# okieraised/rs-face-detection-tflite

Hardware: AMD Instinct MI355X
Metric: faces/sec at batch=256 (256x256 back-camera) per GPU (higher is better)
Workload: dtype f32

## Files before the change

### rs-face-detection-tflite_amd/csrc/chain_kernels.hip

```cpp
#include <hip/hip_runtime.h>

#include <algorithm>
#include <cstdint>
#include <type_traits>

#include "kernels.hpp"
#include "launch.hpp"

namespace mi {

typedef float f32x16c __attribute__((ext_vector_type(16)));
typedef float f32x2c __attribute__((ext_vector_type(2)));
typedef float f32x4c __attribute__((ext_vector_type(4)));

namespace {

__device__ __forceinline__ float4 cld4(const float* p) { return *reinterpret_cast<const float4*>(p); }

struct ChainGeom {
    int Cp, Ch, C4, PS, RS, MT;
    int off_wdw, off_bdw, off_bias, off_alpha;
    int split;
    int pre_P, pre_RP, pre_GP, pre_PS, pre_RS;
    int off_t8;
    int lds_bytes;
    unsigned long long* stamps;
};
#ifdef MI_CHAIN_STAMPS
unsigned long long* g_chain_stamps = nullptr;
#define MI_CHAIN_STAMP(k) if (g.stamps && threadIdx.x == 0) { __builtin_amdgcn_sched_barrier(0); g.stamps[(long)blockIdx.x * 24 + (k)] = __builtin_amdgcn_s_memtime(); __builtin_amdgcn_sched_barrier(0); }
#else
#define MI_CHAIN_STAMP(k)
#endif

constexpr int chain_pre_passes(int C, int H, int W, int Cin, int post_Co, int MT, bool split, long tile) {
    const int pre_RS = (2 * W + 1) * (Cin + 4);
    for (int P = 1; P <= 4; P++) {
        const int RP = (H + P - 1) / P, GP = (RP * W + 31) / 32;
        const long stage = (long)(2 * RP + 1) * pre_RS;
        const long rest = 9 * C + C + 8 * 32 + 64 + (post_Co ? (long)(H >> 1) * (W >> 1) * (post_Co + 4) : 0);
        if ((P - 1) * RP < H && P * GP * (split ? MT : 1) <= 8 && ((stage > tile ? stage : tile) + rest) * 4 <= 160 * 1024 - 256) return P;
    }
    return 0;
}

struct GeomRun {
    [[maybe_unused]] static constexpr bool fixed = false;
    static constexpr bool all_res = false;
    const ChainArgs& a;
    const ChainGeom& g;
    __device__ GeomRun(const ChainArgs& a_, const ChainGeom& g_) : a(a_), g(g_) {}
    __device__ int C() const { return a.C; }
    __device__ int H() const { return a.H; }
    __device__ int W() const { return a.W; }
    __device__ int pre_on() const { return a.pre.on; }
    __device__ int pre_Cin() const { return a.pre.Cin; }
    __device__ int post_on() const { return a.post.on; }
    __device__ int post_Co() const { return a.post.Co; }
#define MI_GEOM_FIELD(f) __device__ int f() const { return g.f; }
    MI_GEOM_FIELD(Cp) MI_GEOM_FIELD(Ch) MI_GEOM_FIELD(C4) MI_GEOM_FIELD(PS) MI_GEOM_FIELD(RS)
    MI_GEOM_FIELD(off_wdw) MI_GEOM_FIELD(off_bdw) MI_GEOM_FIELD(off_bias) MI_GEOM_FIELD(off_alpha)
    MI_GEOM_FIELD(pre_P) MI_GEOM_FIELD(pre_RP) MI_GEOM_FIELD(pre_GP) MI_GEOM_FIELD(pre_PS) MI_GEOM_FIELD(pre_RS)
#undef MI_GEOM_FIELD
};
template <int C_, int H_, int W_, int CIN, int CO>
struct GeomFixed {
    static constexpr bool fixed = true;
    static constexpr bool all_res = true;
    struct K {
        static constexpr int C = C_, H = H_, W = W_, Cp = C, Ch = C / 2, C4 = C / 4, PS = C + 4, RS = (W + 2) * PS, MT = (C + 31) / 32;
        static constexpr bool split = MT > 1 && ((H * W + 31) / 32) * MT <= 8;
        static constexpr int pre_on = CIN != 0, pre_Cin = CIN, post_on = CO != 0, post_Co = CO;
        static constexpr int tile = (H + 2) * RS;
        static constexpr int pre_PS = CIN + 4, pre_RS = (2 * W + 1) * pre_PS;
        static constexpr int pre_P = CIN ? chain_pre_passes(C, H, W, CIN, CO, MT, split, tile) : 0;
        static constexpr int pre_RP = CIN ? (H + pre_P - 1) / pre_P : 0, pre_GP = (pre_RP * W + 31) / 32;
        static constexpr int stage = CIN ? (2 * pre_RP + 1) * pre_RS : 0;
        static constexpr int off_wdw = stage > tile ? stage : tile, off_bdw = off_wdw + 9 * Cp, off_bias = (off_bdw + Cp + 3) & ~3;
        static constexpr int off_alpha = off_bias + MT * 32;
    };
    static_assert(!CIN || K::pre_P > 0, "no staging plan for `pre`");
    __device__ GeomFixed(const ChainArgs&, const ChainGeom&) {}
#define MI_GEOM_FIELD(f) static constexpr __device__ int f() { return K::f; }
    MI_GEOM_FIELD(C) MI_GEOM_FIELD(H) MI_GEOM_FIELD(W) MI_GEOM_FIELD(pre_on) MI_GEOM_FIELD(pre_Cin) MI_GEOM_FIELD(post_on) MI_GEOM_FIELD(post_Co)
    MI_GEOM_FIELD(Cp) MI_GEOM_FIELD(Ch) MI_GEOM_FIELD(C4) MI_GEOM_FIELD(PS) MI_GEOM_FIELD(RS)
    MI_GEOM_FIELD(off_wdw) MI_GEOM_FIELD(off_bdw) MI_GEOM_FIELD(off_bias) MI_GEOM_FIELD(off_alpha)
    MI_GEOM_FIELD(pre_P) MI_GEOM_FIELD(pre_RP) MI_GEOM_FIELD(pre_GP) MI_GEOM_FIELD(pre_PS) MI_GEOM_FIELD(pre_RS)
#undef MI_GEOM_FIELD
    static bool matches(const ChainArgs& a, const ChainGeom& g) {
        bool ok = a.C == K::C && a.H == K::H && a.W == K::W && g.Cp == K::Cp && g.Ch == K::Ch && g.C4 == K::C4 && g.PS == K::PS && g.RS == K::RS &&
                  g.MT == K::MT && (g.split != 0) == K::split && g.off_wdw == K::off_wdw && g.off_bdw == K::off_bdw && g.off_bias == K::off_bias &&
                  g.off_alpha == K::off_alpha && (a.pre.on != 0) == (CIN != 0) && (a.post.on != 0) == (CO != 0);
        if (ok && CIN) ok = a.pre.Cin == CIN && g.pre_P == K::pre_P && g.pre_RP == K::pre_RP && g.pre_GP == K::pre_GP && g.pre_PS == K::pre_PS && g.pre_RS == K::pre_RS;
        if (ok && CO) ok = a.post.Co == CO;
        for (int k = 0; ok && k < a.nblocks; k++) ok = a.blocks[k].has_res != 0;
        return ok;
    }
};
constexpr int kActRun = -1;

struct DwTaps { f32x4c w[9], d[9], b; };
template <int WS_, int RSB_, int PSB_, bool BIAS_FIRST_>
struct DwForm { static constexpr int WS = WS_, RSB = RSB_, PSB = PSB_; static constexpr bool bias_first = BIAS_FIRST_; };
template <int OFF>
__device__ __forceinline__ void lds_request(unsigned addr, f32x4c& v) { asm volatile("ds_read_b128 %0, %1 offset:%2" : "=v"(v) : "v"(addr), "n"(OFF)); }
template <class F, int... K>
__device__ __forceinline__ void dw_request(unsigned wa, unsigned ta, DwTaps& t, std::integer_sequence<int, K...>) {
    static_assert(9 * F::WS + 16 * 16 < 65536 && 2 * F::RSB + 2 * F::PSB + 16 * 16 < 65536, "ds_read offsets are 16 bits");
    ((lds_request<K * F::WS>(wa, t.w[K]), lds_request<(K / 3) * F::RSB + (K % 3) * F::PSB>(ta, t.d[K])), ...);
    lds_request<9 * F::WS>(wa, t.b);
}
template <class F>
__device__ __forceinline__ void dw_request(unsigned wa, unsigned ta, DwTaps& t) { dw_request<F>(wa, ta, t, std::make_integer_sequence<int, 9>{}); }
__device__ __forceinline__ void dw_landed(DwTaps& t) {
    asm volatile("s_waitcnt lgkmcnt(0)" ::: "memory");
#pragma unroll
    for (int k = 0; k < 9; k++) asm volatile("" : "+v"(t.w[k]), "+v"(t.d[k]));
    asm volatile("" : "+v"(t.b));
}
template <bool BIAS_FIRST>
__device__ __forceinline__ void dw_fma(const DwTaps& t, float4& bf) {
    f32x2c lo = {0.f, 0.f}, up = {0.f, 0.f};
    if constexpr (BIAS_FIRST) { lo = f32x2c{t.b.x, t.b.y}; up = f32x2c{t.b.z, t.b.w}; }
#pragma unroll
    for (int k = 0; k < 9; k++) {
        lo = __builtin_elementwise_fma(f32x2c{t.d[k].x, t.d[k].y}, f32x2c{t.w[k].x, t.w[k].y}, lo);
        up = __builtin_elementwise_fma(f32x2c{t.d[k].z, t.d[k].w}, f32x2c{t.w[k].z, t.w[k].w}, up);
    }
    if constexpr (!BIAS_FIRST) { lo += f32x2c{t.b.x, t.b.y}; up += f32x2c{t.b.z, t.b.w}; }
    asm volatile("" : "+v"(lo), "+v"(up));
    bf = make_float4(lo.x, lo.y, up.x, up.y);
}

template <int MT, bool SPLIT, class GP = GeomRun, int ACT = kActRun, int SCHED = 0>
__global__ __launch_bounds__(512, 2) void chain_kernel(ChainArgs a, ChainGeom g) {
    extern __shared__ __attribute__((aligned(16))) float lds[];
    const GP geo(a, g);
    float* tile = lds;
    const int tid = threadIdx.x, lane = tid & 63, wave = tid >> 6;
    const int pl = lane & 31, h = lane >> 5;
    const int b = blockIdx.x;
    const float* in = a.in + (long)b * a.in_fs;
    const int rowf4 = geo.W() * geo.C4();
    const int nch = geo.Ch() >> 2;

    struct ConstRegs { float w[3], bdw, bias, alpha; };
    auto fetch_consts = [&](const ChainBlock& cb, int Cs, int Cos, ConstRegs& r) {
#pragma unroll
        for (int k = 0; k < 3; k++) {
            const int i = tid + 512 * k, c = i % geo.Cp();
            r.w[k] = (i < 9 * geo.Cp() && c < Cs) ? cb.w_dw[(i / geo.Cp()) * Cs + c] : 0.f;
        }
        r.bdw = (tid < Cs && cb.b_dw) ? cb.b_dw[tid] : 0.f;
        r.bias = (tid < Cos && cb.bias) ? cb.bias[tid] : 0.f;
        if constexpr (ACT == kActRun) r.alpha = (tid < Cos && cb.act == ACT_PRELU) ? cb.alpha[tid] : (cb.act == ACT_NONE ? 1.f : 0.f);
    };
    auto commit_consts = [&](const ConstRegs& r) {
#pragma unroll
        for (int k = 0; k < 3; k++)
            if (tid + 512 * k < 9 * geo.Cp()) lds[geo.off_wdw() + tid + 512 * k] = r.w[k];
        if (tid < geo.Cp()) lds[geo.off_bdw() + tid] = r.bdw;
        if (tid < MT * 32) {
            lds[geo.off_bias() + tid] = r.bias;
            if constexpr (ACT == kActRun) lds[geo.off_alpha() + tid] = r.alpha;
        }
    };
    unsigned aoff[MT];
#pragma unroll
    for (int m = 0; m < MT; m++) {
        aoff[m] = (unsigned)((m * nch * 64 + lane) * 4);
        if constexpr (GP::fixed) asm volatile("" : "+v"(aoff[m]));
    }
    auto a_frag = [&](const ChainBlock& cb, int nchk, int j, float4 (&av)[MT]) {
#ifdef MI_ABL_CHAIN_NOA
#pragma unroll
        for (int m = 0; m < MT; m++) { av[m] = make_float4(1.f, 2.f, 3.f, 4.f); asm volatile("" : "+v"(av[m].x), "+v"(av[m].y), "+v"(av[m].z), "+v"(av[m].w)); }
#else
        if constexpr (GP::fixed) {
            if (nchk == nch) {
#pragma unroll
                for (int m = 0; m < MT; m++) av[m] = cld4(cb.w_pw + (long)j * 256 + (size_t)aoff[m]);
                return;
            }
        }
#pragma unroll
        for (int m = 0; m < MT; m++) av[m] = cld4(cb.w_pw + (((long)m * nchk + j) * 64 + lane) * 4);
#endif
// ... 138 lines not shown
                asm volatile("" : "+v"(D1));
                dw_landed(t);
                dw_fma<F::bias_first>(t, bf);
                __builtin_amdgcn_sched_barrier(0);
            }
        }
    };
    auto finish1 = [&](f32x16c& D1, int ch, int gq, const float4& skip, float hi) {
        if constexpr (ACT == ACT_RELU) {
            const f32x2c* bb = reinterpret_cast<const f32x2c*>(lds + geo.off_bias() + ch);
            const f32x2c v0 = (f32x2c{D1[4 * gq], D1[4 * gq + 1]} + bb[0]) + f32x2c{skip.x, skip.y};
            const f32x2c v1 = (f32x2c{D1[4 * gq + 2], D1[4 * gq + 3]} + bb[1]) + f32x2c{skip.z, skip.w};
            D1[4 * gq] = fmaxf(v0.x, 0.f);
            D1[4 * gq + 1] = fmaxf(v0.y, 0.f);
            D1[4 * gq + 2] = fmaxf(v1.x, 0.f);
            D1[4 * gq + 3] = fmaxf(v1.y, 0.f);
            return;
        }
        const float4 bb = cld4(lds + geo.off_bias() + ch), al = cld4(lds + geo.off_alpha() + ch);
        const float4 v = make_float4(D1[4 * gq] + bb.x + skip.x, D1[4 * gq + 1] + bb.y + skip.y, D1[4 * gq + 2] + bb.z + skip.z, D1[4 * gq + 3] + bb.w + skip.w);
        D1[4 * gq] = fminf(fmaxf(v.x, 0.f) + al.x * fminf(v.x, 0.f), hi);
        D1[4 * gq + 1] = fminf(fmaxf(v.y, 0.f) + al.y * fminf(v.y, 0.f), hi);
        D1[4 * gq + 2] = fminf(fmaxf(v.z, 0.f) + al.z * fminf(v.z, 0.f), hi);
        D1[4 * gq + 3] = fminf(fmaxf(v.w, 0.f) + al.w * fminf(v.w, 0.f), hi);
    };
    const float4 zero4 = make_float4(0.f, 0.f, 0.f, 0.f);

    const int ngrp = (geo.H() * geo.W() + 31) >> 5;
    const int grp_w = SPLIT ? wave % ngrp : wave, mt_w = SPLIT ? wave / ngrp : 0;
    const int q = grp_w * 32 + pl;
    const bool valid = q < geo.H() * geo.W();
    const int oy = valid ? q / geo.W() : 0, ox = valid ? q - (q / geo.W()) * geo.W() : 0;
    const bool wave_active = SPLIT ? wave < ngrp * MT : wave * 32 < geo.H() * geo.W();
    const int base0 = oy * geo.RS() + ox * geo.PS() + h * geo.Ch();
    float* centre = tile + (oy + 1) * geo.RS() + (ox + 1) * geo.PS();

    MI_CHAIN_STAMP(0)
    ConstRegs cr;
    if (geo.pre_on()) {
        const ChainBlock& cb = a.pre.blk;
        const int Cin = geo.pre_Cin(), Chp = Cin >> 1, Hi = 2 * geo.H(), Wi = 2 * geo.W(), C4i = Cin >> 2;
        const int PSi = geo.pre_PS(), RSi = geo.pre_RS(), rowf4i = Wi * C4i;
        const float* src = a.pre.in + (long)b * a.pre.in_fs;
        fetch_consts(cb, Cin, geo.C(), cr);
        commit_consts(cr);
        fetch_consts(a.blocks[0], geo.C(), geo.C(), cr);
        const float* wdw = lds + geo.off_wdw();
        const float* bdw = lds + geo.off_bdw();
        f32x16c D[SPLIT ? 1 : MT];
        bool mine = false;
        float* my_centre = tile;
        int my_mt = 0;
        const int UP = SPLIT ? geo.pre_GP() * MT : geo.pre_GP();
        for (int p = 0; p < geo.pre_P(); p++) {
            const int r0 = p * geo.pre_RP(), r1 = min(r0 + geo.pre_RP(), geo.H());
            const int nrows = 2 * (r1 - r0) + 1;
            if (p) __syncthreads();
            for (int i = tid; i < nrows * rowf4i; i += 512) {
                const int rr = i / rowf4i, e = i - rr * rowf4i, px = e / C4i, c4 = e - px * C4i, iy = 2 * r0 + rr;
                *reinterpret_cast<float4*>(lds + rr * RSi + px * PSi + 4 * c4) = iy < Hi ? cld4(src + ((long)iy * rowf4i + e) * 4) : zero4;
            }
            for (int i = tid; i < nrows * C4i; i += 512) {
                const int rr = i / C4i, c4 = i - rr * C4i;
                *reinterpret_cast<float4*>(lds + rr * RSi + Wi * PSi + 4 * c4) = zero4;
            }
            __syncthreads();
            MI_CHAIN_STAMP(16 + p)
            const int u = wave - p * UP;
            if (u >= 0 && u < UP) {
                const int ugrp = SPLIT ? u % geo.pre_GP() : u, umt = SPLIT ? u / geo.pre_GP() : 0;
                const int qp = ugrp * 32 + pl;
                const bool vp = qp < (r1 - r0) * geo.W();
                const int oyl = vp ? qp / geo.W() : 0, oxp = vp ? qp - (qp / geo.W()) * geo.W() : 0;
                const float* t0 = lds + (2 * oyl) * RSi + (2 * oxp) * PSi;
                auto dw = [&](int j, float4& bf) {
                    const int c0 = h * Chp + 4 * j;
                    bf = cld4(bdw + c0);
#pragma unroll
                    for (int ky = 0; ky < 3; ky++)
#pragma unroll
                        for (int kx = 0; kx < 3; kx++) {
                            const float4 w = cld4(wdw + (ky * 3 + kx) * geo.Cp() + c0);
                            const float4 d = cld4(t0 + ky * RSi + kx * PSi + c0);
                            bf.x = fmaf(d.x, w.x, bf.x);
                            bf.y = fmaf(d.y, w.y, bf.y);
                            bf.z = fmaf(d.z, w.z, bf.z);
                            bf.w = fmaf(d.w, w.w, bf.w);
                        }
                };
                if constexpr (SCHED == 1 && !SPLIT) {
                    using K = typename GP::K;
                    contract_ph(DwForm<K::Cp * 4, K::pre_RS * 4, K::pre_PS * 4, true>{}, std::integral_constant<int, K::pre_Cin / 8>{}, cb,
                                lds_addr(wdw + h * Chp), lds_addr(t0 + h * Chp), D);
                } else if constexpr (SPLIT) contract1(cb.w_pw, Chp >> 2, umt, dw, D[0]);
                else contract(cb, Chp >> 2, dw, D);
                const float hi = cb.act == ACT_RELU6 ? 6.f : INFINITY;
#pragma unroll
                for (int m = 0; m < (SPLIT ? 1 : MT); m++)
#pragma unroll
                    for (int gq = 0; gq < 4; gq++) {
                        const int ch = (SPLIT ? umt : m) * 32 + 8 * gq + 4 * h;
                        if (ch >= geo.C()) continue;
                        float4 sk = zero4;
                        if (cb.has_res && ch < Cin) {
                            const float4 s0 = cld4(t0 + ch), s1 = cld4(t0 + PSi + ch), s2 = cld4(t0 + RSi + ch), s3 = cld4(t0 + RSi + PSi + ch);
                            sk = make_float4(fmaxf(fmaxf(s0.x, s1.x), fmaxf(s2.x, s3.x)), fmaxf(fmaxf(s0.y, s1.y), fmaxf(s2.y, s3.y)),
// ... 225 lines not shown
bool make_chain_geom(const ChainArgs& a, ChainGeom* out) {
    ChainGeom g{};
    if (a.C % 8 || a.H * a.W > 256 || a.nblocks < 1 || a.nblocks > kMaxChain) return false;
    g.Cp = a.C; g.Ch = a.C / 2; g.C4 = a.C / 4; g.PS = a.C + 4; g.RS = (a.W + 2) * g.PS;
    g.MT = (a.C + 31) / 32;
    if (g.MT > 4) return false;
    g.split = g.MT > 1 && ((a.H * a.W + 31) / 32) * g.MT <= 8;
    int off = (a.H + 2) * g.RS;
    if (a.pre.on) {
        if (a.pre.Cin % 8 || a.pre.Cin < 8 || a.pre.Cin > a.C) return false;
        g.pre_PS = a.pre.Cin + 4;
        g.pre_RS = (2 * a.W + 1) * g.pre_PS;
        g.pre_P = chain_pre_passes(a.C, a.H, a.W, a.pre.Cin, a.post.on ? a.post.Co : 0, g.MT, g.split != 0, off);
        if (!g.pre_P) return false;
        g.pre_RP = (a.H + g.pre_P - 1) / g.pre_P;
        g.pre_GP = (g.pre_RP * a.W + 31) / 32;
        off = (int)std::max<long>((long)(2 * g.pre_RP + 1) * g.pre_RS, off);
    }
    g.off_wdw = off; off += 9 * g.Cp;
    g.off_bdw = off; off += g.Cp;
    off = (off + 3) & ~3;
    g.off_bias = off; off += g.MT * 32;
    g.off_alpha = off; off += g.MT * 32;
    g.off_t8 = -1;
    for (int hd = 0; hd < kChainHeads; hd++) {
        const ChainHead& H = a.heads[hd];
        if (!H.on) continue;
        if (H.Co_a < 4 || H.Co_a % 4 || H.Co_b < 0 || H.Co_a + H.Co_b > 128 || !H.out_a || (H.Co_b && !H.out_b) || !H.w_pw) return false;
        if ((reinterpret_cast<uintptr_t>(H.out_a) & 15) || (H.out_a_fs & 3) || (reinterpret_cast<uintptr_t>(H.w_pw) & 15)) return false;
        if (H.src == 1) {
            if (!a.post.on) return false;
            if (g.off_t8 < 0) { g.off_t8 = off; off += (a.H >> 1) * (a.W >> 1) * (a.post.Co + 4); }
        }
    }
    g.lds_bytes = off * 4;
    if (g.lds_bytes > 160 * 1024 - 256) return false;
    auto aligned16 = [](const void* p) { return (reinterpret_cast<uintptr_t>(p) & 15) == 0; };
    if (!aligned16(a.in) || !aligned16(a.out) || (a.in_fs & 3) || (a.out_fs & 3)) return false;
    if (a.pre.on && (a.pre.Cin % 8 || a.pre.Cin < 8 || a.pre.Cin > a.C || !aligned16(a.pre.in) || (a.pre.in_fs & 3))) return false;
    if (a.post.on && ((a.H & 1) || (a.W & 1) || a.post.Co % 4 || a.post.Co < a.C || a.post.Co > g.MT * 32 || !aligned16(a.post.out) || (a.post.out_fs & 3))) return false;
    *out = g;
    return true;
}

using Geom16 = GeomFixed<96, 16, 16, 48, 96>;
using Geom8 = GeomFixed<96, 8, 8, 0, 0>;

bool all_relu(const ChainArgs& a) {
    bool ok = (!a.pre.on || a.pre.blk.act == ACT_RELU) && (!a.post.on || a.post.blk.act == ACT_RELU);
    for (int k = 0; ok && k < a.nblocks; k++) ok = a.blocks[k].act == ACT_RELU;
    return ok;
}

template <int MT, bool SPLIT, class GP = GeomRun, int ACT = kActRun, int SCHED = 0>
int launch_chain_inst(const ChainArgs& a, const ChainGeom& g, hipStream_t s) {
    auto kern = chain_kernel<MT, SPLIT, GP, ACT, SCHED>;
    if (hipError_t e = allow_full_lds(reinterpret_cast<const void*>(kern)); e != hipSuccess) return (int)e;
    return (int)launch_kernel(kern, dim3((unsigned)a.B), dim3(512), (size_t)g.lds_bytes, s, a, g);
}

}

bool chain_kernel_supports(const ChainArgs& a) {
    ChainGeom g;
    return make_chain_geom(a, &g);
}

int launch_chain(const ChainArgs& a, void* stream, int fixed, int sched) {
    ChainGeom g;
    if (!make_chain_geom(a, &g)) return (int)hipErrorInvalidValue;
#ifdef MI_CHAIN_STAMPS
    g.stamps = g_chain_stamps;
#endif
    hipStream_t s = (hipStream_t)stream;
    if (fixed && all_relu(a)) {
        if (Geom16::matches(a, g)) return sched ? launch_chain_inst<3, false, Geom16, ACT_RELU, 1>(a, g, s) : launch_chain_inst<3, false, Geom16, ACT_RELU, 0>(a, g, s);
        if (Geom8::matches(a, g)) return sched ? launch_chain_inst<3, true, Geom8, ACT_RELU, 1>(a, g, s) : launch_chain_inst<3, true, Geom8, ACT_RELU, 0>(a, g, s);
    }
    switch (g.MT) {
        case 1: return launch_chain_inst<1, false>(a, g, s);
        case 2: return g.split ? launch_chain_inst<2, true>(a, g, s) : launch_chain_inst<2, false>(a, g, s);
        case 3: return g.split ? launch_chain_inst<3, true>(a, g, s) : launch_chain_inst<3, false>(a, g, s);
        case 4: return g.split ? launch_chain_inst<4, true>(a, g, s) : launch_chain_inst<4, false>(a, g, s);
    }
    return (int)hipErrorInvalidValue;
}

}

#ifdef MI_CHAIN_STAMPS
extern "C" void mi_debug_set_chain_stamps(unsigned long long* p) { mi::g_chain_stamps = p; }
#endif
```

### rs-face-detection-tflite_amd/csrc/engine.cpp

```cpp
#include "engine.hpp"
#include "launch.hpp"

#include <algorithm>
#include <cstdio>
#include <cstdlib>
#include <cstring>
#include <stdexcept>

namespace mi {

void hip_check(hipError_t e, const char* what) {
    if (e != hipSuccess) throw std::runtime_error(std::string(what) + ": " + hipGetErrorString(e));
}

namespace {
template <class T>
void upload(T*& dev, std::vector<T>& host, const char* what_alloc, const char* what_copy) {
    if (dev) hip_check(hipFree(dev), "hipFree");
    dev = nullptr;
    if (host.empty()) return;
    hip_check(hipMalloc(reinterpret_cast<void**>(&dev), host.size() * sizeof(T)), what_alloc);
    hip_check(hipMemcpy(dev, host.data(), host.size() * sizeof(T), hipMemcpyHostToDevice), what_copy);
    std::vector<T>().swap(host);
}
// ... 22 lines not shown
    if (d_arena_) hipFree(d_arena_);
    if (d_small_) hipFree(d_small_);
    if (d_in_stage_) hipFree(d_in_stage_);
    free_bandnet();
    for (float* p : d_out_)
        if (p) hipFree(p);
    for (hipStream_t st : side_streams_) hipStreamDestroy(st);
    for (hipEvent_t ev : lane_events_) hipEventDestroy(ev);
    for (hipStream_t st : head_streams_) hipStreamDestroy(st);
    for (hipEvent_t ev : head_events_) if (ev) hipEventDestroy(ev);
    if (stream_) hipStreamDestroy(stream_);
}

void Model::invalidate_graphs() {
    if (!graphs_.empty()) (void)hipDeviceSynchronize();
    for (auto& kv : graphs_) hipGraphExecDestroy(kv.second);
    graphs_.clear();
}

struct Model::Option {
    enum { kReplan = 1,
           kFreeSmall = 2,
           kKeepGraphs = 4,
           kOneOf = 8,
           kKiB = 16 , kWriteOnly = 32, kReadOnly = 64,
           kBandGen = 128,
           kForms = 256 };
    const char* key;
    int Model::*field;
    int lo, hi, flags;
};

const Model::Option* Model::find_option(const std::string& key) {
    using O = Option;
    constexpr int kMax = 0x7fffffff;
    static const Option table[] = {
        {"chunk", &Model::chunk_, 0, kMax, 0},
        {"graph", &Model::use_graph_, 0, 1, 0},
        {"fuse", &Model::fuse_level_, 0, 5, O::kReplan},
        {"res_budget", &Model::res_budget_, 16, 156, O::kReplan | O::kKiB},
        {"pipe", &Model::pipe_max_, 0, 4, O::kReplan},
        {"small_chain", &Model::small_chain_, 0, 64, O::kFreeSmall},
        {"pipe_rows", &Model::pipe_rows_, 1 << 1 | 1 << 2 | 1 << 4, 0, O::kOneOf},
        {"pipe_band", &Model::pipe_band_, 0, 4096, 0},
        {"strip", &Model::strip_, 0, 1, 0},
        {"stem_fuse", &Model::stem_fuse_, 0, 1, 0},
        {"stem_mfma", &Model::stem_mfma_, 0, 2, O::kForms},
        {"conv_mfma", &Model::conv_mfma_, 0, 1, 0},
        {"stem_run", &Model::stem_run_, 0, 32, 0},
        {"pair_fuse", &Model::pair_fuse_, 0, 1, 0},
        {"mdb_band", &Model::mdb_band_, 0, 4096, 0},
        {"chain_fixed", &Model::chain_fixed_, 0, 1, 0},
        {"chain_sched", &Model::chain_sched_, 0, 1, 0},
        {"mchain", &Model::mchain_, 0, 1, 0},
        {"tail", &Model::tail_, 0, 1, O::kReplan},
        {"tail_pre", &Model::tail_pre_, 0, 2, 0},
        {"tail_g", &Model::tail_g_, 0, 64, 0},
        {"band", &Model::band_, 0, 2, O::kReplan},
        {"band_test_fail", &Model::band_test_fail_, 0, 1, O::kWriteOnly},
        {"band_test_absent", &Model::band_test_absent_, 0, 256, O::kWriteOnly},
        {"band_test_gen", nullptr, 0, kMax, O::kBandGen | O::kWriteOnly},
        {"band_wide", &Model::band_wide_ok_, 0, 1, O::kReplan},
        {"band_fork", &Model::band_fork_, 0, 1, O::kReplan},
        {"band_nw", &Model::band_nw_, 8, 256, O::kReplan},
        {"band_fail_streak", &Model::band_fail_streak_, 0, 0, O::kReadOnly},
        {"band_wraps", &Model::band_wraps_, 0, 0, O::kReadOnly},
        {"fork", &Model::fork_, 0, 1, 0},
        {"heads", &Model::head_streams_opt_, 1, kHeadStreams, O::kReplan},
        {"reuse", &Model::reuse_, 0, 1, O::kReplan},
        {"lanes", &Model::lanes_, 1, 4, 0},
        {"test_poison", &Model::test_poison_, 1 << 1 | 1 << 2, 0, O::kOneOf | O::kKeepGraphs},
    };
    for (const Option& o : table)
        if (key == o.key) return &o;
    return nullptr;
}

void Model::set_option(const std::string& key, int value) {
    const Option* o = find_option(key);
    if (!o || (o->flags & Option::kReadOnly)) throw std::runtime_error("unknown option '" + key + "'");
    int v = (o->lo == 0 && o->hi == 1) ? value != 0 : std::min(o->hi, std::max(o->lo, value));
    if (o->flags & Option::kOneOf) v = (value >= 0 && value < 31 && (o->lo >> value & 1)) ? value : 0;
    if (o->flags & Option::kForms) v = (value >= o->lo && value <= o->hi) ? value : 1;
    if (o->flags & Option::kKiB) v *= 1024;
    if (o->flags & Option::kBandGen) { band_gen_ = static_cast<unsigned>(v); band_gen_force_ = true; }
    else this->*o->field = v;
    if (o->flags & Option::kKeepGraphs) return;
    if (o->flags & Option::kReplan) dirty_ = true;
    if ((o->flags & Option::kFreeSmall) && d_small_) { hipFree(d_small_); d_small_ = nullptr; small_floats_ = 0; }
    invalidate_graphs();
    chunk_cap_ = 0;
}

int Model::get_option(const std::string& key) const {
    const Option* o = find_option(key);
    if (!o || (o->flags & Option::kWriteOnly)) throw std::runtime_error("unknown option '" + key + "'");
    const int v = this->*o->field;
    return (o->flags & Option::kKiB) ? v / 1024 : v;
}

void Model::rebuild() {
    if (d_small_) { hipFree(d_small_); d_small_ = nullptr; small_floats_ = 0; }
    hip_check(hipSetDevice(device_), "hipSetDevice");
    invalidate_graphs();
    plan_ = build_plan(parse_tflite(blob_.data(), blob_.size()), fuse_level_, pipe_max_, res_budget_, tail_ != 0);
    if (!reuse_) {
// ... 138 lines not shown
                const int Cm = g.tensors[m.in[0]].shape[3];
                if (m.kind == Node::Conv) macs += elems(m.out) * m.KH * m.KW * Cm * batch;
                else macs += static_cast<double>(mo[1]) * mo[2] * Cm * ((m.w >= 0 ? 9 : 0) + mo[3]) * batch;
                for (int c : {m.w, m.b, m.w2, m.b2, m.alpha}) bytes += 4 * elems(c);
            }
        }
        if (n.kind == Node::Chain) {
            for (int t : n.extra_out) bytes += 4 * elems(t) * batch;
            for (const Node& m : n.members) {
                const auto& mo = g.tensors[m.out].shape;
                macs += static_cast<double>(mo[1]) * mo[2] * g.tensors[m.in[0]].shape[3] * (9 + mo[3]) * batch;
            }
            for (const Node& m : n.members)
                for (int c : {m.w, m.b, m.w2, m.b2, m.alpha}) bytes += 4 * elems(c);
            for (const Node& m : n.head_nodes) {
                macs += elems(m.out) * g.tensors[m.in[0]].shape[3] * batch;
                for (int c : {m.w, m.b, m.w2, m.b2}) bytes += 4 * elems(c);
            }
        }
        st.bytes += bytes;
        st.macs += macs;
        auto dims = [](const std::vector<int>& sh) {
            std::string d;
            for (size_t q = 1; q < sh.size(); q++) d += (q > 1 ? "x" : "") + std::to_string(sh[q]);
            return d;
        };
        if (static_cast<int>(i) == first.launches[k].node) st.detail = dims(si) + "->";
        st.detail = st.detail.substr(0, st.detail.find("->") + 2) + dims(so);
    }
    return stats;
}

LaunchCtx Model::launch_ctx(const float* in, int chunk_start, int frames) const {
    LaunchCtx c;
    c.weights = d_weights_;
    c.arena = d_arena_ + static_cast<size_t>(plan_.arena_floats_per_frame) * chunk_cap_ * arena_lane_;
    c.in = in; c.out = d_out_.data();
    c.small = d_small_; c.small_floats = small_floats_;
    c.progs = d_programs_; c.tail_progs = d_tail_programs_;
    c.band_prog = d_band_prog_; c.band_consts = d_band_consts_; c.band_ws = d_band_ws_; c.band_sync = d_band_sync_; c.band_fail = d_band_fail_;
    c.chunk_cap = chunk_cap_; c.chunk_start = chunk_start; c.F = frames;
    c.u8_frames = u8_.frames; c.u8_lut = u8_.lut; c.u8_frame_bytes = u8_.frame_bytes; c.u8_row_bytes = u8_.row_bytes;
    c.strip = strip_; c.pair_fuse = pair_fuse_; c.stem_fuse = stem_fuse_; c.stem_mfma = stem_mfma_; c.stem_run = stem_run_; c.mchain = mchain_; c.conv_mfma = conv_mfma_;
    c.small_chain = small_chain_; c.lanes = lanes_;
    c.pipe_rows = pipe_rows_; c.pipe_band = pipe_band_; c.mdb_band = mdb_band_; c.tail_pre = tail_pre_; c.tail_g = tail_g_;
    c.fork = fork_ && lanes_ == 1;
    c.cu_count = device_cu_count();
    c.band = band_use_ && chunk_start == 0;
    c.band_test_absent = band_test_absent_;
    return c;
}

namespace {
int issue(const Launch& l, hipStream_t s, int chain_fixed, int chain_sched) {
    auto many = [&](int (*f)(const BlockArgs*, int, void*)) { return f(l.blocks.data(), static_cast<int>(l.blocks.size()), s); };
    switch (l.to) {
        case Launcher::Conv: return launch_conv(std::get<ConvArgs>(l.args), s);
        case Launcher::HeadGemm: return launch_head_gemm(std::get<HeadGemmArgs>(l.args), s);
        case Launcher::Dw: return launch_dw(std::get<DwArgs>(l.args), s);
        case Launcher::Xc: return launch_xc(std::get<XcArgs>(l.args), s);
        case Launcher::Mdblock: return launch_mdblock(std::get<DblockArgs>(l.args), s);
        case Launcher::Dblock: return launch_dblock(std::get<DblockArgs>(l.args), s);
        case Launcher::Mbneck: return launch_mbneck(std::get<BneckArgs>(l.args), s);
        case Launcher::Bneck: return launch_bneck(std::get<BneckArgs>(l.args), s);
        case Launcher::Tail: return launch_tail(std::get<TailLaunch>(l.args), s);
        case Launcher::Resident: return launch_resident(std::get<ResLaunch>(l.args), s);
        case Launcher::Chain: return launch_chain(std::get<ChainArgs>(l.args), s, chain_fixed, chain_sched);
        case Launcher::StripPipe: return many(launch_strip_pipe);
        case Launcher::MstripChain: return many(launch_mstrip_chain);
        case Launcher::SmallChain: {
            int rc = 0;
            for (size_t k = 0; k < l.blocks.size() && rc == 0; k++) rc = l.blocks[k].sh == 1 ? launch_strip(l.blocks[k], s) : launch_block(l.blocks[k], s);
            return rc;
        }
        case Launcher::Ms2: return launch_ms2(std::get<BlockArgs>(l.args), s);
        case Launcher::Mwalk: return launch_mwalk(std::get<BlockArgs>(l.args), s);
        case Launcher::Strip: return launch_strip(std::get<BlockArgs>(l.args), s);
        case Launcher::Mstrip: return launch_mstrip(std::get<BlockArgs>(l.args), s);
        case Launcher::Block: return launch_block(std::get<BlockArgs>(l.args), s);
        case Launcher::Add: return launch_add(std::get<EltArgs>(l.args), s);
        case Launcher::Act: return launch_act(std::get<EltArgs>(l.args), s);
        case Launcher::Maxpool: return launch_maxpool(std::get<EltArgs>(l.args), s);
        case Launcher::Padc: return launch_padc(std::get<EltArgs>(l.args), s);
        case Launcher::Resize2x: return launch_resize2x(std::get<EltArgs>(l.args), s);
        case Launcher::DepthToSpace: return launch_depth_to_space(std::get<EltArgs>(l.args), s);
        case Launcher::Bandnet: return launch_bandnet(std::get<BandLaunch>(l.args), s);
    }
    return 0;
}
}

void Model::enqueue_chunk(const float* in, int chunk_start, int F, hipStream_t trunk, std::vector<hipEvent_t>* marks, Lowered* keep) {
    LaunchCtx ctx = launch_ctx(in, chunk_start, F);
    if (marks) ctx.fork = false;
    Lowered low = lower_chunk(plan_, consts_, band_plan_, sched_, ctx, keep != nullptr);
    auto mark = [&] {
        if (!marks) return;
        hipEvent_t ev;
        hip_check(hipEventCreate(&ev), "hipEventCreate");
        hip_check(hipEventRecord(ev, trunk), "hipEventRecord");
        marks->push_back(ev);
    };
    mark();
    const size_t n_launches = low.launches.size(), start_event = plan_.nodes.size();
    auto event = [&](size_t k) {
        if (head_events_.size() < plan_.nodes.size() + 2 + kHeadStreams) head_events_.resize(plan_.nodes.size() + 2 + kHeadStreams, nullptr);
        if (!head_events_[k]) hip_check(hipEventCreateWithFlags(&head_events_[k], hipEventDisableTiming), "hipEventCreate");
        return head_events_[k];
    };
    unsigned used_heads = 0;
    for (size_t k = 0; k < n_launches; k++) {
        const Launch& l = low.launches[k];
        hipStream_t s = trunk;
        if (l.slot >= 0) {
            while (static_cast<int>(head_streams_.size()) <= l.slot) {
                hipStream_t st;
                hip_check(hipStreamCreateWithFlags(&st, hipStreamNonBlocking), "hipStreamCreate");
                head_streams_.push_back(st);
            }
            s = head_streams_[static_cast<size_t>(l.slot)];
            if (l.wait >= 0) {
                hip_check(wait_event(s, event(static_cast<size_t>(low.launch_of_node[static_cast<size_t>(l.wait)]))), "hipStreamWaitEvent");
            } else {
                hip_check(record_event(event(start_event), trunk), "hipEventRecord");
                hip_check(wait_event(s, event(start_event)), "hipStreamWaitEvent");
            }
            used_heads |= 1u << l.slot;
        }
        int rc = 0;
        for (int rep = 0; rep < (marks ? profile_inner_ : 1) && rc == 0; rep++) rc = issue(l, s, chain_fixed_, chain_sched_);
        if (rc != 0) throw std::runtime_error(std::string("kernel launch failed: ") + hipGetErrorString(static_cast<hipError_t>(rc)));
        if (l.record) hip_check(record_event(event(k), s), "hipEventRecord");
        mark();
    }
    for (int k = 0; k < kHeadStreams; k++)
        if (used_heads & (1u << k)) {
            hip_check(record_event(event(start_event + 1 + static_cast<size_t>(k)), head_streams_[static_cast<size_t>(k)]), "hipEventRecord");
            hip_check(wait_event(trunk, event(start_event + 1 + static_cast<size_t>(k))), "hipStreamWaitEvent");
        }
    last_chunk_frames_ = F;
    if (keep) *keep = std::move(low);
}

void Model::enqueue_all(const float* in, int batch, hipStream_t s) {
    if (lanes_ > 1 && batch > chunk_cap_) {
        while (static_cast<int>(side_streams_.size()) < lanes_ - 1) {
            hipStream_t st;
            hip_check(hipStreamCreateWithFlags(&st, hipStreamNonBlocking), "hipStreamCreate");
            side_streams_.push_back(st);
        }
        while (static_cast<int>(lane_events_.size()) < lanes_) {
            hipEvent_t ev;
            hip_check(hipEventCreateWithFlags(&ev, hipEventDisableTiming), "hipEventCreate");
            lane_events_.push_back(ev);
        }
        hip_check(record_event(lane_events_[0], s), "hipEventRecord");
        int lane = 0;
        for (int start = 0; start < batch; start += chunk_cap_, lane = (lane + 1) % lanes_) {
            hipStream_t ls = lane == 0 ? s : side_streams_[lane - 1];
            if (lane > 0 && start < chunk_cap_ * lanes_) hip_check(wait_event(ls, lane_events_[0]), "hipStreamWaitEvent");
            arena_lane_ = lane;
            enqueue_chunk(in, start, std::min(chunk_cap_, batch - start), ls);
        }
        arena_lane_ = 0;
        for (int l = 1; l < lanes_; l++) {
            hip_check(record_event(lane_events_[l], side_streams_[l - 1]), "hipEventRecord");
            hip_check(wait_event(s, lane_events_[l]), "hipStreamWaitEvent");
        }
        return;
    }
    int chunk = chunk_cap_;
    for (int start = 0; start < batch; start += chunk) enqueue_chunk(in, start, std::min(chunk, batch - start), s);
}

bool Model::takes_u8_input() {
    if (dirty_) rebuild();
    return mi::takes_u8_input(plan_, consts_);
}

void Model::poison_scratch(hipStream_t s) {
    const int byte = test_poison_ == 1 ? 0xFF : 0x7F;
    if (d_arena_) hip_check(hipMemsetAsync(d_arena_, byte, std::max<size_t>(arena_floats_, 64) * sizeof(float), s), "hipMemsetAsync poison arena");
    if (d_small_) hip_check(hipMemsetAsync(d_small_, byte, small_floats_ * sizeof(float), s), "hipMemsetAsync poison small-batch scratch");
// ... 167 lines not shown
```

### rs-face-detection-tflite_amd/csrc/engine.hpp

```cpp
#pragma once

#include <hip/hip_runtime.h>

#include <map>
#include <memory>
#include <string>
#include <vector>

#include "bandplan.hpp"
#include "consts.hpp"
#include "launches.hpp"
#include "plan.hpp"

namespace mi {

void hip_check(hipError_t e, const char* what);

class Model {
   public:
    Model(const uint8_t* bytes, size_t n, int device);
    ~Model();
    Model(const Model&) = delete;
    Model& operator=(const Model&) = delete;

    int device() const { return device_; }
    const Graph& graph() const { return plan_.graph; }
    const Plan& plan() const { return plan_; }
    std::vector<int> input_dims() const { return plan_.graph.tensors[plan_.graph.inputs[0]].shape; }
    int num_outputs() const { return static_cast<int>(plan_.graph.outputs.size()); }
    const std::vector<int>& output_dims(int i) const { return plan_.graph.tensors[plan_.graph.outputs.at(i)].shape; }
    size_t output_elems(int i) const { return plan_.graph.tensors[plan_.graph.outputs.at(i)].elems(); }
    size_t input_elems() const { return plan_.graph.tensors[plan_.graph.inputs[0]].elems(); }

    void run_device(const float* in, int batch, hipStream_t stream, bool one_shot = false);
    bool band_failed();
    int get_option(const std::string& key) const;
    int band_workgroups(int batch);
    void run(const float* in, int batch, float* const* outs, int mem, hipStream_t stream);
    float* output_device(int i) const { return d_out_.at(i); }
    hipStream_t stream() const { return stream_; }
    bool takes_u8_input();
    void run_device_u8(const uint8_t* frames, long frame_bytes, int row_bytes, const float* lut, int batch, hipStream_t stream);

    struct LaunchStat {
        std::string kernel, detail;
        double ms = 0, bytes = 0, macs = 0;
    };
    std::vector<LaunchStat> profile(const float* in, int batch, int reps, hipStream_t stream);
    void set_option(const std::string& key, int value);
    size_t debug_tensor(int tensor, int frame, float* dst, size_t cap);
    std::string describe() const { return plan_.describe(); }

   private:
    void rebuild();
    struct Option;
    static const Option* find_option(const std::string& key);
    void build_bandnet();
    void free_bandnet();
    bool band_usable(int batch) const;
    void band_before_launch(hipStream_t s);
    void poison_scratch(hipStream_t s);
    void ensure_capacity(int batch);
    LaunchCtx launch_ctx(const float* in, int chunk_start, int frames) const;
    void enqueue_chunk(const float* in, int chunk_start, int frames, hipStream_t s, std::vector<hipEvent_t>* marks = nullptr, Lowered* keep = nullptr);
    void enqueue_all(const float* in, int batch, hipStream_t s);
    void invalidate_graphs();

    int device_ = 0;
    std::vector<uint8_t> blob_;
    Plan plan_;
    int fuse_level_ = 5, pipe_max_ = 4, tail_ = 1, reuse_ = 1;
    int res_budget_ = 156 * 1024;
    int chunk_ = 0, lanes_ = 1, use_graph_ = 1;
    int fork_ = 1, head_streams_opt_ = 1;
    int conv_mfma_ = 1;
    int strip_ = 1, stem_fuse_ = 1, stem_mfma_ = 1, stem_run_ = 0, pair_fuse_ = 1, mchain_ = 1, chain_fixed_ = 1, chain_sched_ = 1;
    int pipe_rows_ = 0, pipe_band_ = 0, mdb_band_ = 0;
    int tail_pre_ = 0, tail_g_ = 0;
    int arena_lane_ = 0;
    std::vector<hipStream_t> side_streams_;
    std::vector<hipEvent_t> lane_events_;
    SideSchedule sched_;
    std::vector<hipStream_t> head_streams_;
    std::vector<hipEvent_t> head_events_;
    bool dirty_ = true;

    float* d_weights_ = nullptr;
    PlanConsts consts_;
    int profile_inner_ = 1;

    ResStage* d_programs_ = nullptr;
    TailStage* d_tail_programs_ = nullptr;
    float* d_arena_ = nullptr;
    size_t arena_floats_ = 0;
    int chunk_cap_ = 0;
    int batch_cap_ = 0;
    std::vector<float*> d_out_;
    float* d_in_stage_ = nullptr;
    size_t in_stage_floats_ = 0;
    int last_chunk_frames_ = 0;

    int band_ = 1;
    int band_nw_ = 128;
    BandPlan band_plan_;
    bool band_use_ = false;
    bool band_ran_ = false;
    int band_test_fail_ = 0;
    int band_test_absent_ = 0;
    int test_poison_ = 0;
    int band_fail_streak_ = 0;
    bool band_disabled_ = false;
    unsigned band_gen_ = 0;
    bool band_gen_force_ = false;
    int band_wraps_ = 0;
    size_t band_ws_bytes_ = 0;
    int band_fork_ = 1, band_wide_ok_ = 1;
    BandPacked* d_band_prog_ = nullptr;
    float* d_band_consts_ = nullptr;
    float* d_band_ws_ = nullptr;
    unsigned* d_band_sync_ = nullptr;
    int* h_band_fail_ = nullptr;
    int* d_band_fail_ = nullptr;

    hipStream_t stream_ = nullptr;
    int small_chain_ = 16;
    float* d_small_ = nullptr;
    size_t small_floats_ = 0;
    struct GraphKey {
        const void* in;
// ... 24 lines not shown
```

### rs-face-detection-tflite_amd/csrc/kernels.hpp

```cpp
#pragma once

#include <cstddef>
#include <cstdint>

namespace mi {

enum ActKind : int { ACT_NONE = 0, ACT_RELU = 1, ACT_RELU6 = 2, ACT_PRELU = 3 };
enum ResMode : int { RES_NONE = 0, RES_DIRECT = 1, RES_MAXPOOL = 2, RES_UP2X = 3 };

struct Epilogue {
    const float* bias = nullptr;
    const float* alpha = nullptr;
    const float* res = nullptr;
    long res_fs = 0;
    int res_mode = RES_NONE;
    int res_C = 0;
    int res_W = 0, res_H = 0;
    int act = ACT_NONE;
    int res_after = 0;
};

struct ConvArgs {
    const float* in = nullptr;
    const uint8_t* in_u8 = nullptr;
// ... 226 lines not shown
    int G = 1;
    int frame_floats = 0;
    int variant = 0;
    ResBases bases;
};
int launch_tail(const TailLaunch& a, void* stream);
bool tail_stage_ok(int kind, int K, int S, int src_C, int Kv, int Co, bool dst_lds);
unsigned tail_magic(int d);

int launch_conv(const ConvArgs& a, void* stream);
const char* conv_kernel_label(const ConvArgs& a);
bool conv_takes_u8(const ConvArgs& a);
bool conv_mfma_shape_ok(int C, int KH, int KW, int Co);
bool conv_mfma_supports(const ConvArgs& a);
int launch_conv_mfma(const ConvArgs& a, void* stream);
int launch_dw(const DwArgs& a, void* stream);
int launch_block(const BlockArgs& a, void* stream);
bool block_kernel_supports(const BlockArgs& a);
const char* block_kernel_label(const BlockArgs& a, char* buf, size_t cap);
int launch_strip(const BlockArgs& a, void* stream);
bool strip_kernel_supports(const BlockArgs& a);
bool strip_shape_ok(int C, int Co);
int strip_consts_floats(int C);
void strip_pack_consts(int C, const float* w_dw, const float* b_dw, const float* w_pw, const float* bias, const float* alpha, int act, float* dst);
const char* strip_kernel_label(const BlockArgs& a, char* buf, size_t cap);
int launch_mwalk(const BlockArgs& a, void* stream);
bool mwalk_kernel_supports(const BlockArgs& a);
bool mwalk_shape_ok(int W, int C, int Co);
int mwalk_consts_floats(int W, int C, int Co);
void mwalk_pack_consts(int W, int C, int Co, const float* w_dw, const float* b_dw, const float* w_pw, const float* bias, const float* alpha, int act, float* dst);
const char* mwalk_kernel_label(const BlockArgs& a, char* buf, size_t cap);
int launch_ms2(const BlockArgs& a, void* stream);
bool ms2_kernel_supports(const BlockArgs& a);
bool ms2_shape_ok(int W, int C, int Co, bool skip);
int ms2_consts_floats(int W, int C, int Co, bool skip);
void ms2_pack_consts(int W, int C, int Co, bool skip, const float* w_dw, const float* b_dw, const float* w_pw, const float* bias, const float* alpha, int act, float* dst);
const char* ms2_kernel_label(const BlockArgs& a, char* buf, size_t cap);
int launch_mstrip(const BlockArgs& a, void* stream);
bool mstrip_kernel_supports(const BlockArgs& a);
bool mstrip_shape_ok(int C, int Co);
int mstrip_consts_floats(int C);
void mstrip_pack_consts(int C, const float* w_dw, const float* b_dw, const float* w_pw, const float* bias, const float* alpha, int act, float* dst);
const char* mstrip_kernel_label(const BlockArgs& a, char* buf, size_t cap);
bool mstrip_chain_supports(const BlockArgs* blocks, int n);
int launch_mstrip_chain(const BlockArgs* blocks, int n, void* stream);
bool strip_pipe_supports(const BlockArgs* blocks, int n);
bool strip_pipe_shape_ok(int C, int W);
bool strip_tail_shape_ok(int C, int Co, int H, int W);
int strip_consts_s2_floats(int C, int Co);
void strip_pack_consts_s2(int C, int Co, const float* w_dw, const float* b_dw, const float* w_pw, const float* bias, const float* alpha, int act, float* dst);
int launch_strip_pipe(const BlockArgs* blocks, int n, void* stream);
const char* strip_pipe_label(const BlockArgs* blocks, int n, char* buf, size_t cap);
int strip_pipe_rows_per_step(int H, int hint = 0);
int launch_chain(const ChainArgs& a, void* stream, int fixed = 1, int sched = 1);

struct BneckBlock {
    const float* w1 = nullptr;
    const float* w2 = nullptr;
    const float* consts = nullptr;
    float hi1 = 0.f, hi2 = 0.f;
    const float* mconsts = nullptr;
    int act1 = ACT_RELU, act2 = ACT_RELU;
};
constexpr int kMaxBneck = 6;
struct BneckArgs {
    const float* in = nullptr;
    float* out = nullptr;
    long in_fs = 0, out_fs = 0;
    int B = 0, H = 0, W = 0, C = 0, Cm = 0, nblocks = 0;
    int bands = 1;
    BneckBlock blocks[kMaxBneck];
};
struct XcStage {
    const float* cblob = nullptr;
    int has_dw = 1;
    const float* w_pw = nullptr;
    int C = 0, Co = 0;
    int act = ACT_RELU;
    int skip = 0;
    const float* res = nullptr;
    long res_fs = 0;
    int res_C = 0, res_W = 0;
};
constexpr int kMaxXc = 8;
struct XcArgs {
    const float* in = nullptr;
    float* out = nullptr;
    long in_fs = 0, out_fs = 0;
    int B = 0, H = 0, W = 0, nstages = 0;
    XcStage st[kMaxXc];
};
bool xc_kernel_supports(const XcArgs& a);
int xc_const_floats(int C, int Co);
int launch_xc(const XcArgs& a, void* stream);
struct DblockArgs {
    const float* in = nullptr;
    float* out = nullptr;
    long in_fs = 0, out_fs = 0;
    int B = 0, H = 0, W = 0, C = 0, Cm = 0;
    int Co = 0;
    int skip1 = 0;
    int skip2_from_a = 0;
    const float* consts = nullptr;
    const float* w1 = nullptr;
    const float* w2 = nullptr;
    float hi1 = 0.f, hi2 = 0.f;
    const float* mconsts = nullptr;
// ... 116 lines not shown
```

Before: 222,700.

## Prefetch pass-1 input rows into registers on idle waves during pass 0

For the fixed 16x16 chain geometry, the two-pass pre-block loop is specialised. Waves that sit idle during pass 0 now load pass 1's input rows from global memory into registers while the other waves compute pass 0. After a barrier those registers are written to LDS, so the serialized global-to-LDS staging before pass 1 is hidden behind compute. It is enabled by default through a new chain_edges option, and it costs extra register pressure (up to 24 float4 per thread) plus a specialised code path that carries static asserts on the geometry.

```diff
diff --git a/rs-face-detection-tflite_amd/csrc/chain_kernels.hip b/rs-face-detection-tflite_amd/csrc/chain_kernels.hip
--- a/rs-face-detection-tflite_amd/csrc/chain_kernels.hip
+++ b/rs-face-detection-tflite_amd/csrc/chain_kernels.hip
@@ -29,8 +29,10 @@
 #ifdef MI_CHAIN_STAMPS
 unsigned long long* g_chain_stamps = nullptr;
 #define MI_CHAIN_STAMP(k) if (g.stamps && threadIdx.x == 0) { __builtin_amdgcn_sched_barrier(0); g.stamps[(long)blockIdx.x * 24 + (k)] = __builtin_amdgcn_s_memtime(); __builtin_amdgcn_sched_barrier(0); }
+#define MI_CHAIN_STAMP_LANDED(k, t) if (g.stamps && threadIdx.x == (t)) { asm volatile("s_waitcnt vmcnt(0)" ::: "memory"); __builtin_amdgcn_sched_barrier(0); g.stamps[(long)blockIdx.x * 24 + (k)] = __builtin_amdgcn_s_memtime(); __builtin_amdgcn_sched_barrier(0); }
 #else
 #define MI_CHAIN_STAMP(k)
+#define MI_CHAIN_STAMP_LANDED(k, t)
 #endif
 
 constexpr int chain_pre_passes(int C, int H, int W, int Cin, int post_Co, int MT, bool split, long tile) {
@@ -132,7 +134,7 @@
     bf = make_float4(lo.x, lo.y, up.x, up.y);
 }
 
-template <int MT, bool SPLIT, class GP = GeomRun, int ACT = kActRun, int SCHED = 0>
+template <int MT, bool SPLIT, class GP = GeomRun, int ACT = kActRun, int SCHED = 0, int EDGES = 0>
 __global__ __launch_bounds__(512, 2) void chain_kernel(ChainArgs a, ChainGeom g) {
     extern __shared__ __attribute__((aligned(16))) float lds[];
     const GP geo(a, g);
@@ -377,6 +379,79 @@
         float* my_centre = tile;
         int my_mt = 0;
         const int UP = SPLIT ? geo.pre_GP() * MT : geo.pre_GP();
+        constexpr bool kRowRegs = EDGES == 1 && SCHED == 1 && !SPLIT;
+        if constexpr (kRowRegs) {
+            using K = typename GP::K;
+            constexpr int UPc = K::pre_GP, NLT = (8 - UPc) * 64, C4c = K::pre_Cin / 4, F4R = 2 * K::W * C4c, NPR = UPc < 8 ? 2 * K::pre_RP * F4R / NLT : 0;
+            static_assert(K::pre_P == 2 && K::H == 2 * K::pre_RP && 2 * UPc <= 8 && 2 * K::pre_RP * F4R == NPR * NLT && NPR <= 24,
+                          "pass 1 = NPR quads for every thread of the waves that are idle in pass 0, which are the waves of pass 1's units");
+            const int wave_s = __builtin_amdgcn_readfirstlane(wave);
+            float4 pr[NPR];
+            auto unit = [&](int p) __attribute__((always_inline)) {
+                const int qp = (wave_s - p * UPc) * 32 + pl;
+                const bool vp = qp < K::pre_RP * K::W;
+                const int oyl = vp ? qp / K::W : 0, oxp = vp ? qp - (qp / K::W) * K::W : 0;
+                const float* t0 = lds + (2 * oyl) * K::pre_RS + (2 * oxp) * K::pre_PS;
+                contract_ph(DwForm<K::Cp * 4, K::pre_RS * 4, K::pre_PS * 4, true>{}, std::integral_constant<int, K::pre_Cin / 8>{}, cb,
+                            lds_addr(wdw + h * Chp), lds_addr(t0 + h * Chp), D);
+                const float hi = cb.act == ACT_RELU6 ? 6.f : INFINITY;
+#pragma unroll
+                for (int m = 0; m < MT; m++)
+#pragma unroll
+                    for (int gq = 0; gq < 4; gq++) {
+                        const int ch = m * 32 + 8 * gq + 4 * h;
+                        if (ch >= K::C) continue;
+                        float4 sk = make_float4(0.f, 0.f, 0.f, 0.f);
+                        if (cb.has_res && ch < K::pre_Cin) {
+                            const float4 s0 = cld4(t0 + ch), s1 = cld4(t0 + K::pre_PS + ch), s2 = cld4(t0 + K::pre_RS + ch), s3 = cld4(t0 + K::pre_RS + K::pre_PS + ch);
+                            sk = make_float4(fmaxf(fmaxf(s0.x, s1.x), fmaxf(s2.x, s3.x)), fmaxf(fmaxf(s0.y, s1.y), fmaxf(s2.y, s3.y)),
+                                             fmaxf(fmaxf(s0.z, s1.z), fmaxf(s2.z, s3.z)), fmaxf(fmaxf(s0.w, s1.w), fmaxf(s2.w, s3.w)));
+                        }
+                        finish1(D[m], ch, gq, sk, hi);
+                    }
+                mine = vp;
+                my_centre = tile + (p * K::pre_RP + oyl + 1) * K::RS + (oxp + 1) * K::PS;
+            };
+            for (int i = tid; i < (2 * K::pre_RP + 1) * F4R; i += 512) {
+                const int rr = i / F4R, e = i - rr * F4R, px = e / C4c, c4 = e - px * C4c;
+                *reinterpret_cast<float4*>(lds + rr * K::pre_RS + px * K::pre_PS + 4 * c4) = cld4(src + 4 * (long)i);
+            }
+            for (int i = tid; i < (2 * K::pre_RP + 1) * C4c; i += 512) {
+                const int rr = i / C4c, c4 = i - rr * C4c;
+                *reinterpret_cast<float4*>(lds + rr * K::pre_RS + 2 * K::W * K::pre_PS + 4 * c4) = zero4;
+            }
+            __syncthreads();
+            MI_CHAIN_STAMP(16)
+            if (wave_s < UPc) {
+                unit(0);
+            } else {
+                const float* s1 = src + 4 * ((long)(2 * K::pre_RP) * F4R + (tid - UPc * 64));
+#pragma unroll
+                for (int k = 0; k < NPR; k++) pr[k] = cld4(s1 + 4 * NLT * k);
+                MI_CHAIN_STAMP_LANDED(18, UPc * 64)
+            }
+            MI_CHAIN_STAMP(19)
+            __syncthreads();
+            if (wave_s >= UPc) {
+#pragma unroll
+                for (int k = 0; k < NPR; k++) {
+                    const int i = tid - UPc * 64 + NLT * k, rr = i / F4R, e = i - rr * F4R, px = e / C4c, c4 = e - px * C4c;
+                    *reinterpret_cast<float4*>(lds + rr * K::pre_RS + px * K::pre_PS + 4 * c4) = pr[k];
+                }
+            } else {
+                for (int i = tid; i < F4R; i += UPc * 64) {
+                    const int px = i / C4c, c4 = i - px * C4c;
+                    *reinterpret_cast<float4*>(lds + 2 * K::pre_RP * K::pre_RS + px * K::pre_PS + 4 * c4) = zero4;
+                }
+                for (int i = tid; i < (2 * K::pre_RP + 1) * C4c; i += UPc * 64) {
+                    const int rr = i / C4c, c4 = i - rr * C4c;
+                    *reinterpret_cast<float4*>(lds + rr * K::pre_RS + 2 * K::W * K::pre_PS + 4 * c4) = zero4;
+                }
+            }
+            __syncthreads();
+            MI_CHAIN_STAMP(17)
+            if (wave_s >= UPc && wave_s < 2 * UPc) unit(1);
+        } else
         for (int p = 0; p < geo.pre_P(); p++) {
             const int r0 = p * geo.pre_RP(), r1 = min(r0 + geo.pre_RP(), geo.H());
             const int nrows = 2 * (r1 - r0) + 1;
@@ -708,9 +783,9 @@
     return ok;
 }
 
-template <int MT, bool SPLIT, class GP = GeomRun, int ACT = kActRun, int SCHED = 0>
+template <int MT, bool SPLIT, class GP = GeomRun, int ACT = kActRun, int SCHED = 0, int EDGES = 0>
 int launch_chain_inst(const ChainArgs& a, const ChainGeom& g, hipStream_t s) {
-    auto kern = chain_kernel<MT, SPLIT, GP, ACT, SCHED>;
+    auto kern = chain_kernel<MT, SPLIT, GP, ACT, SCHED, EDGES>;
     if (hipError_t e = allow_full_lds(reinterpret_cast<const void*>(kern)); e != hipSuccess) return (int)e;
     return (int)launch_kernel(kern, dim3((unsigned)a.B), dim3(512), (size_t)g.lds_bytes, s, a, g);
 }
@@ -722,7 +797,7 @@
     return make_chain_geom(a, &g);
 }
 
-int launch_chain(const ChainArgs& a, void* stream, int fixed, int sched) {
+int launch_chain(const ChainArgs& a, void* stream, int fixed, int sched, int edges) {
     ChainGeom g;
     if (!make_chain_geom(a, &g)) return (int)hipErrorInvalidValue;
 #ifdef MI_CHAIN_STAMPS
@@ -730,7 +805,10 @@
 #endif
     hipStream_t s = (hipStream_t)stream;
     if (fixed && all_relu(a)) {
-        if (Geom16::matches(a, g)) return sched ? launch_chain_inst<3, false, Geom16, ACT_RELU, 1>(a, g, s) : launch_chain_inst<3, false, Geom16, ACT_RELU, 0>(a, g, s);
+        if (Geom16::matches(a, g)) {
+            if (sched && edges) return launch_chain_inst<3, false, Geom16, ACT_RELU, 1, 1>(a, g, s);
+            return sched ? launch_chain_inst<3, false, Geom16, ACT_RELU, 1>(a, g, s) : launch_chain_inst<3, false, Geom16, ACT_RELU, 0>(a, g, s);
+        }
         if (Geom8::matches(a, g)) return sched ? launch_chain_inst<3, true, Geom8, ACT_RELU, 1>(a, g, s) : launch_chain_inst<3, true, Geom8, ACT_RELU, 0>(a, g, s);
     }
     switch (g.MT) {
diff --git a/rs-face-detection-tflite_amd/csrc/engine.cpp b/rs-face-detection-tflite_amd/csrc/engine.cpp
--- a/rs-face-detection-tflite_amd/csrc/engine.cpp
+++ b/rs-face-detection-tflite_amd/csrc/engine.cpp
@@ -98,6 +98,7 @@
         {"mdb_band", &Model::mdb_band_, 0, 4096, 0},
         {"chain_fixed", &Model::chain_fixed_, 0, 1, 0},
         {"chain_sched", &Model::chain_sched_, 0, 1, 0},
+        {"chain_edges", &Model::chain_edges_, 0, 1, 0},
         {"mchain", &Model::mchain_, 0, 1, 0},
         {"tail", &Model::tail_, 0, 1, O::kReplan},
         {"tail_pre", &Model::tail_pre_, 0, 2, 0},
@@ -342,7 +343,7 @@
 }
 
 namespace {
-int issue(const Launch& l, hipStream_t s, int chain_fixed, int chain_sched) {
+int issue(const Launch& l, hipStream_t s, int chain_fixed, int chain_sched, int chain_edges) {
     auto many = [&](int (*f)(const BlockArgs*, int, void*)) { return f(l.blocks.data(), static_cast<int>(l.blocks.size()), s); };
     switch (l.to) {
         case Launcher::Conv: return launch_conv(std::get<ConvArgs>(l.args), s);
@@ -355,7 +356,7 @@
         case Launcher::Bneck: return launch_bneck(std::get<BneckArgs>(l.args), s);
         case Launcher::Tail: return launch_tail(std::get<TailLaunch>(l.args), s);
         case Launcher::Resident: return launch_resident(std::get<ResLaunch>(l.args), s);
-        case Launcher::Chain: return launch_chain(std::get<ChainArgs>(l.args), s, chain_fixed, chain_sched);
+        case Launcher::Chain: return launch_chain(std::get<ChainArgs>(l.args), s, chain_fixed, chain_sched, chain_edges);
         case Launcher::StripPipe: return many(launch_strip_pipe);
         case Launcher::MstripChain: return many(launch_mstrip_chain);
         case Launcher::SmallChain: {
@@ -418,7 +419,7 @@
             used_heads |= 1u << l.slot;
         }
         int rc = 0;
-        for (int rep = 0; rep < (marks ? profile_inner_ : 1) && rc == 0; rep++) rc = issue(l, s, chain_fixed_, chain_sched_);
+        for (int rep = 0; rep < (marks ? profile_inner_ : 1) && rc == 0; rep++) rc = issue(l, s, chain_fixed_, chain_sched_, chain_edges_);
         if (rc != 0) throw std::runtime_error(std::string("kernel launch failed: ") + hipGetErrorString(static_cast<hipError_t>(rc)));
         if (l.record) hip_check(record_event(event(k), s), "hipEventRecord");
         mark();
diff --git a/rs-face-detection-tflite_amd/csrc/engine.hpp b/rs-face-detection-tflite_amd/csrc/engine.hpp
--- a/rs-face-detection-tflite_amd/csrc/engine.hpp
+++ b/rs-face-detection-tflite_amd/csrc/engine.hpp
@@ -74,7 +74,7 @@
     int chunk_ = 0, lanes_ = 1, use_graph_ = 1;
     int fork_ = 1, head_streams_opt_ = 1;
     int conv_mfma_ = 1;
-    int strip_ = 1, stem_fuse_ = 1, stem_mfma_ = 1, stem_run_ = 0, pair_fuse_ = 1, mchain_ = 1, chain_fixed_ = 1, chain_sched_ = 1;
+    int strip_ = 1, stem_fuse_ = 1, stem_mfma_ = 1, stem_run_ = 0, pair_fuse_ = 1, mchain_ = 1, chain_fixed_ = 1, chain_sched_ = 1, chain_edges_ = 1;
     int pipe_rows_ = 0, pipe_band_ = 0, mdb_band_ = 0;
     int tail_pre_ = 0, tail_g_ = 0;
     int arena_lane_ = 0;
diff --git a/rs-face-detection-tflite_amd/csrc/kernels.hpp b/rs-face-detection-tflite_amd/csrc/kernels.hpp
--- a/rs-face-detection-tflite_amd/csrc/kernels.hpp
+++ b/rs-face-detection-tflite_amd/csrc/kernels.hpp
@@ -302,7 +302,7 @@
 int launch_strip_pipe(const BlockArgs* blocks, int n, void* stream);
 const char* strip_pipe_label(const BlockArgs* blocks, int n, char* buf, size_t cap);
 int strip_pipe_rows_per_step(int H, int hint = 0);
-int launch_chain(const ChainArgs& a, void* stream, int fixed = 1, int sched = 1);
+int launch_chain(const ChainArgs& a, void* stream, int fixed = 1, int sched = 1, int edges = 1);
 
 struct BneckBlock {
     const float* w1 = nullptr;
```

After: 223,200, median of 6. No clear change (+0.3%).
